# koszullab/instaGRAAL

Measured on AMD Instinct MI355X. Metric: MCMC moves/s (accepted+rejected) at fixed n_frags x nnz, higher is better.
Workload: dtype f32 screening tier with a rigorous bound (every column) + f64 terms (f32 inputs) for the contenders / exact i64 fixed-point sums; 1 GPU; synthetic Hi-C 50k bins / 50M contacts (149003 sub-frags), level 4, 5 neighbours, nuisance sampling off; seed=0, step=one batch of 128 moves (step_sampler calls), moves_warmup=640, parallelism=1 GPU, parameters=synthetic

## Files before the change

### include/instagraal_hip.h

```cpp
#ifndef INSTAGRAAL_HIP_H
#define INSTAGRAAL_HIP_H

#include <stdint.h>

#ifdef __cplusplus
extern "C" {
#endif

#define IG_N_TMP_STRUCT 24
#define IG_MAX_CANDIDATES 16
#define IG_N_INSERT_BLOCKS 6

typedef struct ig_ctx ig_ctx;

typedef struct ig_move_result {
    double o;
    double dist;
    double mean_len;
    int32_t op_sampled;
    int32_t id_f_sampled;
    int32_t n_contigs;
    int32_t n_candidates;
    int64_t n_slice;
    int64_t n_evals;
// ... 17 lines not shown
int ig_set_insert_config(ig_ctx* ctx, const int32_t list_bounds[IG_N_INSERT_BLOCKS], int32_t max_bounds_insert);
int ig_set_initial_genome(ig_ctx* ctx, const int32_t* init_prev, const int32_t* init_next, const int32_t* orientable,
                          const int32_t* blacklisted, int32_t n_blacklisted);

int ig_full_likelihood(ig_ctx* ctx, int which_params, int use_prev_tables, double* nz, double* z, int64_t* limbs5);

int ig_score_move(ig_ctx* ctx, int32_t frag_a, const int32_t* cands, int32_t C, double* scores);
int ig_apply(ig_ctx* ctx, int32_t frag_a, int32_t frag_b, int32_t op);
int ig_step(ig_ctx* ctx, int32_t frag_a, const int32_t* cands, int32_t C, ig_move_result* out, double* scores_or_null);
int ig_step_batch(ig_ctx* ctx, int32_t n_moves, const int32_t* frags, const int32_t* cands, int32_t max_c,
                  ig_move_result* results);
typedef struct ig_neighbours ig_neighbours;
int ig_neighbours_create(const int64_t* indptr, const int32_t* xk, const float* pk, int32_t n_frags, const int32_t* blacklisted,
                         int32_t n_blacklisted, ig_neighbours** out);
void ig_neighbours_destroy(ig_neighbours* nb);
int ig_neighbours_draw(ig_neighbours* nb, uint32_t* mt_key624, int32_t* mt_pos, const int32_t* frags, int32_t n_moves,
                       int32_t n_neighbours, int32_t* cands_out);
int ig_neighbours_draw_nuisance(ig_neighbours* nb, uint32_t* mt_key624, int32_t* mt_pos, int32_t* has_gauss, double* gauss,
                                const int32_t* frags, int32_t n_moves, int32_t n_neighbours, int32_t skip_normal_3, int32_t* cands_out,
                                int32_t* id_modif_out, double* normal_out, double* uniform_out);
int ig_step_draw(ig_ctx* ctx, ig_neighbours* nb, uint32_t* mt_key624, int32_t* mt_pos, int32_t frag_a, int32_t n_neighbours,
                 int32_t* cands, int32_t* n_cands, ig_move_result* out, double* scores_or_null);
int ig_step_batch_draw(ig_ctx* ctx, ig_neighbours* nb, uint32_t* mt_key624, int32_t* mt_pos, int32_t n_moves, const int32_t* frags,
                       int32_t n_neighbours, int32_t* cands_out, ig_move_result* results);
int ig_batch_max_width(ig_ctx* ctx, int32_t max_c);
int ig_batch_upload(ig_ctx* ctx, int32_t n_moves, const int32_t* frags, const int32_t* cands, int32_t max_c, int32_t max_w);
int ig_batch_score(ig_ctx* ctx, int32_t move0, int32_t W, int32_t slot_begin, int32_t slot_end);
int ig_batch_records(ig_ctx* ctx, void** records, int64_t* bytes_per_slot);
int ig_batch_commit(ig_ctx* ctx, int32_t move0, int32_t W, int32_t* n_committed);
int ig_batch_results(ig_ctx* ctx, int32_t n_moves, ig_move_result* results);
int ig_set_batch_width(int w);
int ig_set_window(int w);
int ig_batch_stats(ig_ctx* ctx, int64_t out4[4]);
int ig_scratch_bytes(ig_ctx* ctx, int64_t out3[3]);

int ig_nuis_begin(ig_ctx* ctx, int32_t frag_a, const int32_t* cands, int32_t C, const float p_test[8], float mean_subfrag_kb);
int ig_nuis_end(ig_ctx* ctx, ig_move_result* out, double* nz_test, double* z_test, int64_t* limbs5);
int ig_nuis_accept(ig_ctx* ctx);
int ig_links_inverse(ig_ctx* ctx);
int ig_set_nuis_width(int w);
int ig_nuis_run_begin(ig_ctx* ctx, int32_t n_moves, const int32_t* frags, const int32_t* cands, int32_t max_c);
int ig_nuis_step_begin(ig_ctx* ctx, int32_t move, const float p_test[8], float mean_subfrag_kb);
int ig_nuis_step_next(ig_ctx* ctx, double temperature, double u, const float p_next_rejected[8], const float p_next_accepted[8],
                      float mean_subfrag_kb, int32_t has_next, ig_move_result* out, double* nz_test, double* z_test, int32_t* accepted);
int ig_set_nuis_screen(int on);
int ig_set_nuis_hist(int on);
int ig_set_nuis_chain(int on);
int ig_nuis_chain_begin(ig_ctx* ctx, int32_t move, int32_t n_sets, const float* p_tests, const double* u, const double* temperature,
                        float mean_subfrag_kb);
int ig_nuis_chain_done(ig_ctx* ctx);
int ig_nuis_chain_end(ig_ctx* ctx, int32_t* n_done, int32_t* reason);
int ig_nuis_exact_result(ig_ctx* ctx, double* nz_test);

int ig_renumber_contigs(ig_ctx* ctx, int32_t* n_contigs, float* mean_len, int32_t* max_id);
int ig_bomb(ig_ctx* ctx, const int32_t* shuffle);
int ig_genome_distance(ig_ctx* ctx, double* d);
int ig_get_valid_insert(ig_ctx* ctx, int32_t out12[12]);

int ig_contact_map_order(ig_ctx* ctx, int32_t* order_M, int32_t* n_placed);
int ig_contact_map(ig_ctx* ctx, int32_t max_side, int64_t* image, int64_t image_capacity, int32_t* side, int32_t* bin);

int ig_distance_law(ig_ctx* ctx, const float* edges, int32_t n_edges, int64_t* observed, int64_t* pairs, int64_t scalars[8]);

int ig_set_shard(ig_ctx* ctx, int32_t rank, int32_t world);
int64_t ig_partials_count(ig_ctx* ctx);
void* ig_partials_device_ptr(ig_ctx* ctx);
// ... 39 lines not shown
```

### instagraal_amd/csrc/ig_common.cuh

```cuda
#pragma once

#include <hip/hip_runtime.h>

#include <algorithm>
#include <atomic>
#include <cstdarg>
#include <cstdio>
#include <cstdlib>
#include <cstring>
#include <numeric>
#include <string>
#include <vector>

#include "../../include/ig_detmath.h"
#include "../../include/instagraal_hip.h"
#include "ig_ops.cuh"

#define NSLOT 25
#define NCODE 8
#define NFRESH 4
#define LGF_TAB 1024
#define SCORE_THREADS 256

static thread_local std::string g_err;
// ... 11 lines not shown
#define HIPCK(x)                                                                                     \
    do {                                                                                             \
        hipError_t e_ = (x);                                                                         \
        if (e_ != hipSuccess) return fail("%s failed: %s (%s:%d)", #x, hipGetErrorString(e_), __FILE__, __LINE__); \
    } while (0)


struct SubTab {
    int parent;
    float wat, cri;
    int w;
};

struct State {
    int *pos, *spos, *cid, *sbp, *circ, *prev, *next, *L, *SL, *LB, *ori;
    int *lb, *sl, *sub_first, *rep, *activ, *id_d;
};
#define NDYN 11

struct Tables {
    float* dist;
    float* stot;
    int* len;
    int2* cp;
};

struct CandMeta {
    int B, ctgA, ctgB, same, windowed;
    int LA, LB, SLA, SLB, n_loc, m_loc;
    int lA, lB;
    int n_uniq, uniq[24], kidx[NSLOT];
    int flags[12], pos_up[6], pos_down[6];
    int pos_fa, pos_fb, up_fa, down_fa, up_fb, down_fb;
};

struct ColMeta {
    float stot;
    int len;
};

struct Glob {
    ig_params par[2];
    float mean_kb;
    int slice_nb;
    int list_bounds[6];
    long long nz_hi, nz_lo, z_hi, z_lo, n_intra;
    long long credit2, credit2_acc;
    double n_tot_pxl;
    double lgf[15];
    int n_contigs, next_cid, n_black, N, M;
    int max_L, max_SL;
    int n_prev_touched;
    int valid_insert[12];
    int error;
    int stamp_ctr;
    int retry_pool;
    int retry_pad;
    long long scr_cols, scr_cont;
    long long scr_void_cols;
    long long scr_terms, scr_terms_exact;
    int dbg[8];
};

#define IG_MAX_BATCH 64
struct MoveCtl {
    int A, C, force_slot, fresh;
    int ch_c, ch_k, ch_slot, ch_windowed;
    int superset0;
    int overflow;
    int n_dirty, pad;
    int exact_chunk, pad2;
    double ch_score;
    long long n_slice_tot, n_eval_tot, bytes_min;
    long long d_hi, d_lo;
    long long nzb_hi, nzb_lo;
    int pred, pred_c, pred_k, pred_pad;
    long long pd_hi, pd_lo;
};

struct SlotPre {
    long long nz_hi, nz_lo;
    double nz_d, nz_cut_d;
    long long dz_hi, dz_lo, dni;
    int k;
    unsigned info;
};
struct CandPre {
    long long ext_hi, ext_lo;
    double ext_d;
    long long n_slice;
    int r;
    int base_cnt;
    int ctgA, ctgB, m_loc, n_loc, n_uniq, B;
// ... 319 lines not shown
```

### instagraal_amd/csrc/ig_host_batch.inc

```


static int ensure_io(ig_ctx* c, int n_moves, int max_c)
{
    const size_t need = (size_t)n_moves * (sizeof(int) + (size_t)IG_MAX_CANDIDATES * sizeof(int) + sizeof(ig_move_result));
    if (c->h_stage_bytes < need) {
        if (c->h_stage) hipHostFree(c->h_stage);
        c->h_stage = nullptr;
        c->h_stage_bytes = 0;
        const size_t want = std::max(need, (size_t)1 << 20);
        if (hipHostMalloc((void**)&c->h_stage, want, hipHostMallocDefault) == hipSuccess) c->h_stage_bytes = want;
        else (void)hipGetLastError();
    }
    if (c->results_cap < n_moves) {
        const int cap = std::max(n_moves, 8192);
        hipFree(c->d_results);
        hipFree(c->d_frags);
        DALLOC(c->d_results, (size_t)cap);
        DALLOC(c->d_frags, (size_t)cap);
        c->results_cap = cap;
    }
    if ((long long)c->cands_cap < (long long)n_moves * max_c) {
        const long long cap = std::max((long long)n_moves * max_c, 8192LL * IG_MAX_CANDIDATES);
        hipFree(c->d_cands);
        DALLOC(c->d_cands, (size_t)cap);
// ... 111 lines not shown
    } stale_guard(c, par_only && pb > 0);
    const int N = c->N;
    const int gN = std::max((N + 255) / 256, W);
    const PzTab pz{c->pz_tab, c->pz_n};
    if (phase == 0 || phase == 2) {
        const int n_tw = (c->M + 31) / 32 + 1;
        if (!par_only) {
            c->touched_flip ^= 1;
            c->mb.touched = c->touched_bits + (size_t)c->touched_flip * n_tw;
        }
        if (!par_only) {
            const int mean_len0 = c->n_contigs_seen > 0 ? c->N / c->n_contigs_seen : 0;
            c->mb.nseg = mean_len0 >= 600 ? SLICE_SEG : 8;
        }
        if (!par_only) {
            TimedLaunch t(c, T_GATHER);
            hipLaunchKernelGGL(k_gather, dim3(gN), dim3(256), 0, c->stream, c->st, c->glob, c->mb, c->d_cands, c->d_frags, move0, W, max_c,
                               c->tab, c->tab_prev, c->prev_touched, force_slot, c->touched_bits + (size_t)(c->touched_flip ^ 1) * n_tw, n_tw);
        }
        if (!par_only) {
            TimedLaunch t(c, T_MUTATE);
            c->own_begin = w_begin;
            c->own_end = w_end;
            if (nW > 0) {
                const int mean_len = c->n_contigs_seen > 0 ? c->N / c->n_contigs_seen : 0;
                const int mutate_threads = mean_len >= 600 ? 1024 : (mean_len >= 150 ? 512 : 256);
                hipLaunchKernelGGL(k_mutate, dim3(NSLOT, max_c, nW), dim3(mutate_threads), 0, c->stream, c->st, c->tab, c->sub_tab, c->rowptr,
                                   c->glob, c->mb, pz, w_begin);
            }
        }
        if (force_slot < 0 && nW > 0) {
            if (!par_only) {
                TimedLaunch t(c, T_SLICE);
                hipLaunchKernelGGL(k_offsets, dim3(1), dim3(OFFSETS_THREADS), 0, c->stream, c->mb, W, w_begin, w_end, max_c);
                const int rb_auto = c->n_contigs_seen > 0
                                        ? std::min(SLICE_RB, std::max(32, (int)(2.0 * (double)c->Z / (double)c->n_contigs_seen / 2100.0)))
                                        : SLICE_RB;
                const int rb = nW == 1 ? std::max(rb_auto, 192) : rb_auto;
                const int s_share = 1, s_maxj = 1 << 20;
                if (c->mb.packed)
                    hipLaunchKernelGGL(k_slice<true>, dim3(rb, max_c + 1, nW), dim3(256), 0, c->stream, c->rowptr, c->cc, c->tab, c->glob, c->mb, c->rank,
                                       c->world, w_begin, s_share, s_maxj);
                else
                    hipLaunchKernelGGL(k_slice<false>, dim3(rb, max_c + 1, nW), dim3(256), 0, c->stream, c->rowptr, c->cc, c->tab, c->glob, c->mb, c->rank,
                                       c->world, w_begin, s_share, s_maxj);
            }
            if (par_only && nWp > 0)
                hipLaunchKernelGGL(k_rescore_prepare, dim3(NSLOT, max_c, nWp), dim3(256), 0, c->stream, c->glob, c->mb, pz, pb);
            if (nWp > 0) {
            const int s_screen = getenv("IG_SCREEN") ? atoi(getenv("IG_SCREEN")) : 1;
            const int verify = getenv("IG_SCREEN_VERIFY") ? atoi(getenv("IG_SCREEN_VERIFY")) : 0;
            const bool exact_once = c->exact_next && !par_only;
            if (exact_once) c->exact_next = false;
            const bool screen = (s_screen || verify) && phase == 2 && (W > 1 || c->screen_w1) && c->world == 1 && c->mb.packed && !exact_once;
            c->tail_fused = screen;
            if (phase == 2 && !c->tail_fused) {
                hipEventRecord(c->ev_slice, c->stream);
                hipStreamWaitEvent(c->stream2, c->ev_slice, 0);
                hipLaunchKernelGGL(k_tail, dim3(max_c, nWp), dim3(256), 0, c->stream2, c->rowptr, c->cc, c->tab, c->glob, c->mb, c->lgf_tab,
                                   g_tail_quirk, pz, pb);
                hipEventRecord(c->ev_tail, c->stream2);
            }
            int contenders_only = 0;
            if (screen) {
                const int ny = (NSLOT + 1) / 2;
                const int use_order = (!par_only && pb == w_begin && pe == w_end && nWp * max_c <= (int)OFFSETS_THREADS) ? 1 : 0;
                const int nseg = c->mb.nseg;
                const int Q = std::max(1, std::min(8, (7000 + nseg * ny * max_c * nWp - 1) / (nseg * ny * max_c * nWp)));
                {
                    TimedLaunch t(c, T_SCREEN);
                    const int tsplit = (nWp == 1 && !par_only) ? 6 : 1;
                    if (c->tail_fused)
                        hipLaunchKernelGGL(k_screen_tail, dim3(max_c * nWp * tsplit + nseg * Q * ny * max_c * nWp), dim3(SCORE_THREADS), 0, c->stream,
                                           c->screen_const, c->mb, c->mb.scr, c->mb.scr_void, c->mb.scr_ub, max_c, pb, max_c * nWp * tsplit, c->rowptr, c->cc,
                                           c->tab, c->glob, c->lgf_tab, g_tail_quirk, pz, use_order, Q, tsplit);
                    else
                        hipLaunchKernelGGL(k_screen<0>, dim3(nseg * Q, ny, max_c * nWp), dim3(SCORE_THREADS), 0, c->stream, c->screen_const,
                                           c->mb, c->mb.scr, c->mb.scr_void, c->mb.scr_ub, max_c, pb, use_order, Q);
// ... 639 lines not shown
    if (n_moves < 0 || n_moves > c->up_moves) return fail("ig_batch_results: out of range");
    return download_results(c, n_moves, results);
}

extern "C" int ig_set_batch_width(int w)
{
    g_batch_w = std::min(std::max(w, 1), IG_MAX_BATCH);
    return 0;
}

extern "C" int ig_scratch_bytes(ig_ctx* c, int64_t out3[3])
{
    IG_JOIN(c);
    const MoveBuf& m = c->mb;
    const int64_t C = (int64_t)m.capC * m.capW;
    out3[0] = C * ((int64_t)m.sN * 4 * 3 + (int64_t)m.sM * 4 * 2 + (int64_t)m.sM * NSLOT * 8 + (int64_t)NSLOT * NDYN * m.sN * 4);
    out3[1] = m.pool_cap * (m.packed ? 8 : 12);
    out3[2] = C * (int64_t)(SLICE_SEG * 16 + sizeof(CandMeta) + NSLOT * NCODE * sizeof(ColMeta) + (P_STRIDE + Q_STRIDE) * 8 + IG_N_TMP_STRUCT * 8 +
                            NSLOT * 8 + NSLOT * 16 + 16) +
              (int64_t)m.rec_stride * m.capW + (int64_t)m.work_cap * 8 + (int64_t)c->N * 8;
    return 0;
}

extern "C" int ig_batch_stats(ig_ctx* c, int64_t out3[4])
{
    IG_JOIN(c);
    out3[0] = c->n_batches;
    out3[1] = c->n_batch_committed;
    out3[2] = c->n_batch_pending;
    out3[3] = c->n_batch_predicted;
    return 0;
}

extern "C" int ig_step(ig_ctx* c, int32_t frag_a, const int32_t* cands, int32_t C, ig_move_result* out, double* scores)
{
    IG_JOIN(c);
    HIPCK(hipSetDevice(c->device));
    if (check_ready(c)) return -1;
    if (c->world > 1) return fail("ig_step: this handle scores a contact shard (ig_set_shard %d/%d): partial sums only -- use ig_step_begin / all-reduce / ig_step_finish", c->rank, c->world);
    if (validate_move(c, frag_a, cands, C)) return -1;
    if (ensure_move_buffers(c, std::max(8, (int)C))) return -1;
    if (ensure_io(c, 1, C)) return -1;
    char* stg = (c->h_stage && c->h_stage_bytes >= 8192) ? (char*)c->h_stage : nullptr;
    int* s_in = stg ? (int*)stg : nullptr;
    ig_move_result* s_res = stg ? (ig_move_result*)(stg + 256) : out;
    double* s_sc = stg ? (double*)(stg + 512) : scores;
    if (s_in) {
        s_in[0] = frag_a;
        for (int i = 0; i < C; i++) s_in[1 + i] = cands[i];
    }
    HIPCK(hipMemcpyAsync(c->d_frags, s_in ? (const void*)s_in : (const void*)&frag_a, sizeof(int), hipMemcpyHostToDevice, c->stream));
    HIPCK(hipMemcpyAsync(c->d_cands, s_in ? (const void*)(s_in + 1) : (const void*)cands, (size_t)C * sizeof(int), hipMemcpyHostToDevice, c->stream));
    for (;;) {
        enqueue_move(c, 0, C, -1, 2);
        if (scores) HIPCK(hipMemcpyAsync(s_sc, c->mb.scores, (size_t)C * IG_N_TMP_STRUCT * sizeof(double), hipMemcpyDeviceToHost, c->stream));
        enqueue_apply(c, 0, 0, 0);
        HIPCK(hipMemcpyAsync(s_res, c->d_results, sizeof(ig_move_result), hipMemcpyDeviceToHost, c->stream));
        if (queue_max_readback(c)) return -1;
        HIPCK(hipStreamSynchronize(c->stream));
        if (s_res->pad != 1) break;
        take_max_readback(c);
        if (retry_with_larger_pool(c)) return -1;
    }
    if (stg) {
        *out = *s_res;
        if (scores) memcpy(scores, s_sc, (size_t)C * IG_N_TMP_STRUCT * sizeof(double));
// ... 280 lines not shown
```

### instagraal_amd/csrc/ig_kernels_score.cuh

```cuda
#pragma once


#define CW(w, c) (PS(w) * mb.capC + (c))

__device__ inline int build_uniq(int* u, bool first, int LA, int LB, const int* vf)
{
    int n = 0;
    if (first) {
        u[n++] = 0;
        u[n++] = 1;
    }
    u[n++] = 2;
    u[n++] = 3;
    if (LB != 1)
        for (int k = 4; k < 8; k++) u[n++] = k;
    if (LA != 1)
        for (int k = 8; k < 12; k++) u[n++] = k;
    for (int k = 12; k < IG_N_TMP_STRUCT; k++)
        if (!vf || vf[k - 12] != -1) u[n++] = k;
    return n;
}

__global__ void __launch_bounds__(256)
    k_gather(State st, Glob* g, MoveBuf mb, const int* __restrict__ cands_all, const int* __restrict__ frags_all, int move0, int W,
// ... 281 lines not shown
        for (int x = threadIdx.x; x < n; x += blockDim.x) {
            const int f = S.gid[x];
            ch |= (S.pos[x] != st.pos[f]) | (S.spos[x] != st.spos[f]) | (S.cid[x] != st.cid[f]) | (S.sbp[x] != st.sbp[f]) |
                  (S.circ[x] != st.circ[f]) | (S.prev[x] != st.prev[f]) | (S.next[x] != st.next[f]) | (S.L[x] != st.L[f]) |
                  (S.SL[x] != st.SL[f]) | (S.LB[x] != st.LB[f]) | (S.ori[x] != st.ori[f]);
            hd += (S.pos[x] == 0);
            if (in_lds) {
#pragma unroll
                for (int a = 0; a < NDYN; a++) base[(size_t)a * N + x] = s_loc[a * MUT_LDS_N + x];
            }
        }
        __shared__ int sh_ch, sh_hd;
        if (threadIdx.x == 0) {
            sh_ch = 0;
            sh_hd = 0;
        }
        __syncthreads();
        hd = wave_sum_i(hd);
        if ((threadIdx.x & 63) == 0 && hd) atomicAdd(&sh_hd, hd);
        if (ch) atomicOr(&sh_ch, 1);
        __syncthreads();
        if (threadIdx.x == 0) {
            mb.sinfo[cw * NSLOT + slot] = make_int2(sh_ch, sh_hd);
            if (sh_ch && k > 0) atomicOr(&mb.livecol[cw], 1u << k);
        }
    }
    const ig_params p = g->par[0];
    const float mean = g->mean_kb;
    uint2* col = mb.coords + (size_t)(cw * NSLOT + k) * M;
    ColMeta* cm = mb.cmeta + (size_t)(cw * NSLOT + k) * NCODE;
    int* subs = mb.subs + (size_t)cw * M;
    long long hi = 0, lo = 0, ni = 0;
    __shared__ long long seg_bound[SLICE_SEG];
    if (threadIdx.x < SLICE_SEG) seg_bound[threadIdx.x] = 0;
    __syncthreads();
    for (int x = threadIdx.x; x < n; x += blockDim.x) {
        const int f = S.gid[x];
        const int cid = S.cid[x];
        const int code = (cid == m.ctgA) ? 0 : ((cid == m.ctgB) ? 1 : 2 + (cid - fresh));
        const int ori = S.ori[x], sp = S.spos[x], sl = S.sl[x], SLc = S.SL[x];
        const float stot = (float)(int)((float)S.circ[x] * (float)S.LB[x] / 1000.0f);
        if (S.pos[x] == 0) {
            cm[code].stot = stot;
            cm[code].len = SLc;
        }
        const float sbp_kb = (float)S.sbp[x] / 1000.0f;
        const int sf = st.sub_first[f];
        const int lbase = (x < m.LA) ? 0 : m.SLA;
        for (int q = 0; q < sl; q++) {
            const int s = sf + q;
            const SubTab b = sub[s];
            const float dist = sbp_kb + ((ori == 1) ? b.wat : b.cri);
            const int npos = (ori == 1) ? sp + q : sp + sl - (q + 1);
            const int ls = lbase + tab.cp[s].y;
            uint2 v;
            v.x = __float_as_uint(dist);
            v.y = (unsigned)npos | ((unsigned)code << 28);
            col[ls] = v;
            if (k == 0) {
                subs[ls] = s;
                mb.rowcnt[(size_t)cw * M + ls] = 0;
                const long long rb = rowptr[s], re = rowptr[s + 1];
                atomicAdd((unsigned long long*)&seg_bound[ls & (mb.nseg - 1)], (unsigned long long)(re - rb));
                mb.rowbe[(size_t)cw * M + ls] = make_int4((int)(unsigned)rb, (int)(rb >> 32), (int)(re - rb), s);
            }
            if (npos == 0) ni += ((long long)SLc * (long long)(SLc - 1)) / 2;
            if (npos > 0) {
                const long long q2 = zero_q(p, npos, SLc, stot, mean, pz.v, pz.n);
                hi += q2 >> 32;
                lo += (long long)(unsigned int)q2;
            }
        }
    }
    __shared__ long long red[4][16];
    hi = wave_sum_ll(hi);
    lo = wave_sum_ll(lo);
    ni = wave_sum_ll(ni);
    const int wv = threadIdx.x >> 6;
    if ((threadIdx.x & 63) == 0) {
        red[0][wv] = hi;
        red[1][wv] = lo;
        red[2][wv] = ni;
    }
    __syncthreads();
    if (threadIdx.x == 0) {
        long long* q = mb.qpart + (size_t)cw * Q_STRIDE;
        long long s0 = 0, s1 = 0, s2 = 0;
        for (int v = 0; v < (int)(blockDim.x >> 6); v++) {
            s0 += red[0][v];
            s1 += red[1][v];
            s2 += red[2][v];
        }
        q[Q_Z + 2 * k] = s0;
        q[Q_Z + 2 * k + 1] = s1;
        q[Q_NI + k] = s2;
    }
    if (k == 0 && threadIdx.x < SLICE_SEG) mb.slbound[(size_t)cw * SLICE_SEG + threadIdx.x] = seg_bound[threadIdx.x];
}

__global__ void __launch_bounds__(1024) k_mutate(State st, Tables tab, const SubTab* __restrict__ sub, const long long* __restrict__ rowptr,
                                                Glob* g, MoveBuf mb, PzTab pz, int w_begin)
{
    if (KEPT(w_begin + (int)blockIdx.z)) return;
    mutate_one(st, tab, sub, rowptr, g, mb, pz, blockIdx.x, blockIdx.y, w_begin + blockIdx.z);
}

__global__ void __launch_bounds__(256) k_mutate_winners(State st, Tables tab, const SubTab* __restrict__ sub,
                                                        const long long* __restrict__ rowptr, Glob* g, MoveBuf mb, PzTab pz, int w_start,
                                                        int own_begin, int own_end, const int* __restrict__ batch_out)
{
    const int w = blockIdx.y;
    const int committed = batch_out[0], pending = batch_out[1];
    if (w >= own_begin && w < own_end) return;
    if (!((w >= w_start && w < committed) || w == pending)) return;
    const MoveCtl& mc = mb.ctl[PS(w)];
    if (blockIdx.x == 1 && mc.ch_slot == IG_N_TMP_STRUCT) return;
    mutate_one(st, tab, sub, rowptr, g, mb, pz, blockIdx.x == 0 ? IG_N_TMP_STRUCT : mc.ch_slot, mc.ch_c, w);
}

#define OFFSETS_THREADS 1024
__global__ void __launch_bounds__(OFFSETS_THREADS) k_offsets(MoveBuf mb, int W, int w_begin, int w_end, int max_c)
{
    __shared__ long long wave_tot[OFFSETS_THREADS / 64];
    __shared__ long long s_tot[IG_MAX_BATCH * IG_MAX_CANDIDATES];
    const int tid = threadIdx.x, lane = tid & 63, wv = tid >> 6;
    const int n_idx = (w_end - w_begin) * max_c;
    const bool can_order = n_idx <= IG_MAX_BATCH * IG_MAX_CANDIDATES && n_idx <= (int)OFFSETS_THREADS;
    long long my_tot = 0;
    if (can_order && tid < n_idx) {
        const int w = w_begin + tid / max_c, c = tid % max_c;
        const bool used = c < mb.ctl[PS(w)].C && !KEPT(w);
        for (int sg = 0; sg < SLICE_SEG; sg++) {
            const long long b = mb.slbound[(size_t)CW(w, c) * SLICE_SEG + sg];
            my_tot += (used && b > 0) ? b : 0;
        }
    }
    const int n = W * mb.capC * SLICE_SEG;
    const int per = (n + OFFSETS_THREADS - 1) / OFFSETS_THREADS;
    auto phys = [&](int i) -> size_t {
        const int cwl = i / SLICE_SEG;
        return (size_t)CW(cwl / mb.capC, cwl % mb.capC) * SLICE_SEG + (size_t)(i % SLICE_SEG);
    };
    auto bound_of = [&](int i) -> long long {
        const int cwl = i / SLICE_SEG;
        const int w = cwl / mb.capC, c = cwl % mb.capC;
        return (w >= w_begin && w < w_end && !KEPT(w) && c < mb.ctl[PS(w)].C) ? mb.slbound[phys(i)] : -1;
    };
    constexpr int PER_MAX = (IG_MAX_BATCH * IG_MAX_CANDIDATES * SLICE_SEG + OFFSETS_THREADS - 1) / OFFSETS_THREADS;
    long long bq[PER_MAX];
    __shared__ int s_over[IG_MAX_BATCH];
    if (tid < IG_MAX_BATCH) s_over[tid] = 0;
    long long sum = 0;
#pragma unroll
    for (int q = 0; q < PER_MAX; q++) {
        const int i = tid * per + q;
        bq[q] = (q < per && i < n) ? bound_of(i) : -1;
        sum += bq[q] > 0 ? bq[q] : 0;
    }
    long long incl = sum;
    for (int off = 1; off < 64; off <<= 1) {
        const long long o = __shfl_up(incl, off, 64);
        if (lane >= off) incl += o;
    }
    if (lane == 63) wave_tot[wv] = incl;
    __syncthreads();
    long long run = incl - sum;
    for (int q = 0; q < wv; q++) run += wave_tot[q];
#pragma unroll
    for (int q = 0; q < PER_MAX; q++) {
        const int i = tid * per + q;
        const long long b = bq[q];
        if (b >= 0) {
            if (run + b > mb.pool_cap) {
                mb.sloff[phys(i)] = -1;
                mb.ctl[PS(i / SLICE_SEG / mb.capC)].overflow = 1;
                s_over[i / SLICE_SEG / mb.capC] = 1;
            } else {
                mb.sloff[phys(i)] = run;
            }
            run += b;
        }
    }
    __syncthreads();
#pragma unroll
    for (int q = 0; q < PER_MAX; q++) {
        const int i = tid * per + q;
        if (bq[q] >= 0 && s_over[i / SLICE_SEG / mb.capC]) mb.sloff[phys(i)] = -1;
    }
    if (can_order) {
        if (tid < n_idx) s_tot[tid] = my_tot;
        __syncthreads();
        if (tid < n_idx) {
            int rank = 0;
            for (int u = 0; u < n_idx; u++) rank += (s_tot[u] > my_tot) || (s_tot[u] == my_tot && u < tid);
            mb.order[rank] = ((w_begin + tid / max_c) << 8) | (tid % max_c);
        }
        const int n_slots = w_end - w_begin;
        long long st = 0;
        if (tid < n_slots)
            for (int cc2 = 0; cc2 < max_c; cc2++) st += s_tot[tid * max_c + cc2];
        __syncthreads();
        if (tid < n_slots) s_tot[tid] = st;
        __syncthreads();
        if (tid < n_slots) {
            int rank = 0;
            for (int u = 0; u < n_slots; u++) rank += (s_tot[u] > st) || (s_tot[u] == st && u < tid);
            mb.order[mb.capC * mb.capW + rank] = w_begin + tid;
        }
    } else if (tid < w_end - w_begin) {
        mb.order[mb.capC * mb.capW + tid] = w_begin + tid;
    }
}

#define LDS_COL_CAP 4096
#define DELTA_RB 128

#ifndef SLICE_RB
#define SLICE_RB 96
#endif
#ifndef SLICE_UNROLL
#define SLICE_UNROLL 4
#endif
#ifndef SLICE_MIN_WAVES
#define SLICE_MIN_WAVES 8
#endif
template <bool PACKED>
__global__ void __launch_bounds__(256, SLICE_MIN_WAVES) k_slice(const long long* __restrict__ rowptr, const int2* __restrict__ cc, Tables tab,
                                                                 Glob* g, MoveBuf mb, int rank, int world, int w_begin, int share_rows, int max_j)
{
    const int w = mb.order[mb.capC * mb.capW + blockIdx.z];
    if (KEPT(w)) return;
    const bool shared_plane = (blockIdx.y == 0);
    const int cand_plane = (int)blockIdx.y - 1;
    __shared__ long long seg_off[IG_MAX_CANDIDATES][SLICE_SEG];
    __shared__ int s_cw[IG_MAX_CANDIDATES], s_ctgB[IG_MAX_CANDIDATES], s_idx[IG_MAX_CANDIDATES], s_nc;
    __shared__ int a_same[IG_MAX_CANDIDATES], a_ctgB[IG_MAX_CANDIDATES], a_SLA, a_ctgA, a_mloc[IG_MAX_CANDIDATES];
    const int lane = threadIdx.x & 63, wv = threadIdx.x >> 6;
    const unsigned long long lt_mask = (1ull << lane) - 1ull;
    const int C = mb.ctl[PS(w)].C;
    const int capC = min(mb.capC, IG_MAX_CANDIDATES);
    if ((int)threadIdx.x < capC) {
        const CandMeta& mt = mb.meta[CW(w, threadIdx.x)];
        a_same[threadIdx.x] = mt.same;
        a_ctgB[threadIdx.x] = mt.ctgB;
        a_mloc[threadIdx.x] = mt.m_loc;
        if (threadIdx.x == 0) {
            a_SLA = mt.SLA;
            a_ctgA = mt.ctgA;
        }
    }
    for (int i = threadIdx.x; i < capC * SLICE_SEG; i += blockDim.x) seg_off[i / SLICE_SEG][i % SLICE_SEG] = mb.sloff[(size_t)CW(w, i / SLICE_SEG) * SLICE_SEG + i % SLICE_SEG];
    __syncthreads();
    if (threadIdx.x == 0) {
        int nc = 0;
        if (shared_plane) {
            if (share_rows)
                for (int c = 0; c < C; c++)
                    if (!a_same[c]) {
                        s_idx[nc] = c;
                        s_cw[nc] = CW(w, c);
                        s_ctgB[nc++] = a_ctgB[c];
                    }
        } else if (cand_plane < C) {
            s_idx[0] = cand_plane;
            s_cw[0] = CW(w, cand_plane);
            s_ctgB[0] = a_ctgB[cand_plane];
            nc = 1;
        }
        s_nc = nc;
    }
    __syncthreads();
    const int nc = s_nc;
    if (nc == 0) return;
    if (seg_off[0][0] < 0) return;
    const int cw0 = s_cw[0], c0 = s_idx[0];
    const CandMeta& m = mb.meta[cw0];
    const int M = mb.sM;
    const bool m_same = a_same[c0] != 0;
    const bool own_all = !shared_plane && (m_same || !share_rows);
    const int SLA = a_SLA, ctgA = a_ctgA;
    const int row_lo = (shared_plane || own_all) ? 0 : SLA;
    const int n_rows = shared_plane ? SLA : (a_mloc[c0] - row_lo);
    const int4* rowbe = mb.rowbe + (size_t)cw0 * M;
    const int ctgB0 = s_ctgB[0];
    const int nrw = gridDim.x * 4;
    const int J = min(max_j, max(1, nrw / max(n_rows, 1)));
    for (int item = blockIdx.x * 4 + wv; item < n_rows * J; item += nrw) {
        const int r = row_lo + item % n_rows, j = item / n_rows;
        const int seg = r & (mb.nseg - 1);
        const int4 be = rowbe[r];
        const long long b = (long long)(unsigned)be.x | ((long long)be.y << 32), e = b + be.z;
        const bool in_a = m_same || r < SLA;
        const int2 cp1 = make_int2(in_a ? ctgA : ctgB0, in_a ? r : r - SLA);
        const bool mine = (world <= 1) || ((r % world) == rank);
        int rc = 0;
        if (b != e) {
            for (long long q0 = b + (long long)j * 64 * SLICE_UNROLL; q0 < e; q0 += (long long)J * 64 * SLICE_UNROLL) {
                int2 v[SLICE_UNROLL], cp2[SLICE_UNROLL];
#pragma unroll
                for (int u = 0; u < SLICE_UNROLL; u++) {
                    const long long qi = q0 + u * 64 + lane;
                    v[u] = (qi < e) ? cc[qi] : make_int2(-1, 0);
                }
#pragma unroll
                for (int u = 0; u < SLICE_UNROLL; u++) {
                    const bool hit = (v[u].x >= 0) && ((mb.touched[v[u].x >> 5] >> (v[u].x & 31)) & 1u);
                    cp2[u] = hit ? tab.cp[v[u].x] : make_int2(-1, -1);
                }
                for (int k = 0; k < nc; k++) {
                    bool keep[SLICE_UNROLL];
                    unsigned long long mask[SLICE_UNROLL];
                    int add = 0;
                    const int ctgB = s_ctgB[k];
#pragma unroll
                    for (int u = 0; u < SLICE_UNROLL; u++) {
                        if (own_all) keep[u] = (v[u].x >= 0) && slice_keep(m, cp1.x, cp2[u].x, cp1.y, cp2[u].y, v[u].y, false);
                        else keep[u] = (v[u].x >= 0) && (v[u].y > 0) && ((cp2[u].x == ctgA) || (cp2[u].x == ctgB));
                        mask[u] = __ballot(keep[u]);
                        add += __popcll(mask[u]);
                    }
                    if (!add) continue;
                    rc += (lane == k) ? add : 0;
                    if (!mine) continue;
                    unsigned long long base = 0;
                    if (lane == 0) base = atomicAdd((unsigned long long*)(mb.part + (size_t)s_cw[k] * P_STRIDE + P_CNT + seg), (unsigned long long)add);
                    base = __shfl(base, 0, 64);
                    const long long off = seg_off[s_idx[k]][seg];
                    int o2 = 0;
#pragma unroll
                    for (int u = 0; u < SLICE_UNROLL; u++) {
                        if (keep[u]) {
                            const long long at = off + (long long)base + o2 + __popcll(mask[u] & lt_mask);
                            const int lj = ((m_same || cp2[u].x == ctgA) ? 0 : SLA) + cp2[u].y;
                            if (PACKED) {
                                mb.sl_pk[at] = (unsigned long long)r | ((unsigned long long)lj << 20) | ((unsigned long long)v[u].y << 40);
                            } else {
                                mb.sl_li[at] = r;
                                mb.sl_lj[at] = lj;
                                mb.sl_ob[at] = v[u].y;
                            }
                        }
                        o2 += __popcll(mask[u]);
                    }
                }
            }
        }
        if (lane < nc && rc) atomicAdd(&mb.rowcnt[(size_t)s_cw[lane] * M + r], rc);
    }
}

#define LDS_PZ 1024
#define LDS_LGF 256

__device__ __noinline__ double term_general(const ig_params p, float mean_kb, float s, int dkey, int ob, double lgf, PzTab pz)
{
    const ig_hot h = ig_hot_make(p, ig_tab());
    const int inter = dkey < 0;
    const float ex_z = inter ? p.v_inter : pz_lookup(pz, p, mean_kb, dkey);
    if (h.fast && ob > 0) return ig_term_hot(s, inter, ob, lgf, ex_z, &h, ig_tab());
    const float ex = inter ? p.v_inter : ig_rippe(s, p, ig_tab());
    return ig_pixel_term(ex, ex_z, ob, lgf, ig_tab());
}

__device__ __forceinline__ void quantize_split(double t, int& qh, unsigned& ql)
{
    t = (t != t) ? 0.0 : t;
// ... 1322 lines not shown
```

### instagraal_amd/hip_lib.py

```python
from __future__ import annotations

import ctypes as C
import os
import subprocess

import numpy as np

HERE = os.path.dirname(os.path.abspath(__file__))
ROOT = os.path.dirname(HERE)
LIB_PATH = os.path.join(HERE, "libinstagraal_hip.so")
SRC = os.path.join(HERE, "csrc", "ig_hip.hip")
SRC_HOST = os.path.join(HERE, "csrc", "ig_draw.cpp")
DEPS = [SRC, SRC_HOST] + [os.path.join(HERE, "csrc", f) for f in ("ig_ops.cuh", "ig_common.cuh", "ig_model.cuh", "ig_kernels_setup.cuh",
                                                          "ig_kernels_score.cuh", "ig_kernels_screen.cuh", "ig_kernels_commit.cuh",
                                                          "ig_kernels_nuis.cuh", "ig_kernels_map.cuh", "ig_kernels_law.cuh", "ig_host_core.inc", "ig_host_upload.inc",
                                                          "ig_host_map.inc", "ig_host_law.inc",
                                                          "ig_host_batch.inc", "ig_host_nuis.inc", "ig_host_debug.inc")] + \
       [os.path.join(ROOT, "include", f) for f in ("ig_detmath.h", "ig_detmath_tables.h", "instagraal_hip.h")]

N_TMP_STRUCT = 24
MAX_CANDIDATES = 16

FRAG_FIELDS = ("pos", "sub_pos", "id_c", "start_bp", "len_bp", "sub_len", "circ", "id", "prev", "next", "l_cont",
               "sub_l_cont", "l_cont_bp", "ori", "rep", "activ", "id_d")
# ... 483 lines not shown
        o = np.zeros(12, np.float64)
        _ck(lib().ig_debug_nuis_screen_stats(self._h, _p(o)))
        n = max(o[0] - o[3], 1.0)
        return dict(screened=int(o[0]), rejected_screened=int(o[1]), exact_passes=int(o[2]), void=int(o[3]), largest_bound=float(o[4]),
                    largest_used_fraction=float(o[5]), mean_bound=float(o[6] / n), undecided=int(o[7]),
                    void_why=dict(parameters=int(o[8]), contact=int(o[9]), sums=int(o[10]), no_record=int(o[11])))

    def debug_nuis_hist_stats(self):
        o = np.zeros(12, np.float64)
        _ck(lib().ig_debug_nuis_hist_stats(self._h, _p(o)))
        n = max(o[0] - o[3], 1.0)
        return dict(evaluated=int(o[0]), rejected=int(o[1]), accepted=int(o[2]), void=int(o[3]), mean_bound=float(o[4] / n),
                    largest_used_fraction=float(o[5]), walks=int(o[6]), builds=int(o[7]),
                    void_why=dict(parameters=int(o[8]), contact=int(o[9]), sums=int(o[10]), no_record=int(o[11])))

    def debug_zero_fallbacks(self):
        n = C.c_int64()
        _ck(lib().ig_debug_zero_fallbacks(self._h, C.byref(n)))
        return int(n.value)

    def debug_pool_retries(self):
        n = C.c_int64()
        _ck(lib().ig_debug_pool_retries(self._h, C.byref(n)))
        return int(n.value)

    def debug_nuis_hist_check(self):
        n = C.c_int64()
        _ck(lib().ig_debug_nuis_hist_check(self._h, C.byref(n)))
        return int(n.value)

    def batch_stats(self):
        o = np.zeros(4, np.int64)
        _ck(lib().ig_batch_stats(self._h, _p(o)))
        return dict(batches=int(o[0]), committed_in_batch=int(o[1]), one_move_tails=int(o[2]), predicted_deltas=int(o[3]))

    def scratch_bytes(self):
        o = np.zeros(3, np.int64)
        _ck(lib().ig_scratch_bytes(self._h, _p(o)))
        return int(o[0]), int(o[1]), int(o[2])

    def contact_map_order(self):
        out = np.zeros(max(self.M, 1), np.int32)
        n = C.c_int32()
        _ck(lib().ig_contact_map_order(self._h, _p(out), C.byref(n)))
        return out[:n.value].copy()

    def contact_map(self, max_side):
        from .contact_map import binning

        max_side = int(max_side)
        if not 1 <= max_side <= 2 ** 31 - 1:
            raise HipError("contact_map: max_side must be >= 1 (got %d)" % max_side)
        cap = min(max_side, max(self.M, 1))
        if cap * cap > 1 << 26:
            cap = max(binning(self.contact_map_order().size, max_side)[1], 1)
        img = np.empty(cap * cap, np.int64)
        side, b = C.c_int32(), C.c_int32()
        _ck(lib().ig_contact_map(self._h, C.c_int32(max_side), _p(img), C.c_int64(img.size), C.byref(side), C.byref(b)))
        n = side.value
        return img[:n * n].reshape(n, n).copy(), b.value

    def debug_contact_map_time(self, max_side, combine=True, n=1):
        ms = np.zeros(int(n), np.float32)
        tot = C.c_int64()
        _ck(lib().ig_debug_contact_map_time(self._h, C.c_int32(int(max_side)), C.c_int32(int(bool(combine))), C.c_int32(int(n)), _p(ms),
                                            C.byref(tot)))
        return ms, int(tot.value)
# ... 139 lines not shown
```

Measured before the change: 51960 moves/s.

## Share slice row walks among candidates with same target contig, add walk stats

```diff
diff --git a/include/instagraal_hip.h b/include/instagraal_hip.h
--- a/include/instagraal_hip.h
+++ b/include/instagraal_hip.h
@@ -73,6 +73,7 @@
 int ig_set_batch_width(int w);
 int ig_set_window(int w);
 int ig_batch_stats(ig_ctx* ctx, int64_t out4[4]);
+int ig_slice_walk_stats(ig_ctx* ctx, int64_t out2[2]);
 int ig_scratch_bytes(ig_ctx* ctx, int64_t out3[3]);
 
 int ig_nuis_begin(ig_ctx* ctx, int32_t frag_a, const int32_t* cands, int32_t C, const float p_test[8], float mean_subfrag_kb);
diff --git a/instagraal_amd/csrc/ig_common.cuh b/instagraal_amd/csrc/ig_common.cuh
--- a/instagraal_amd/csrc/ig_common.cuh
+++ b/instagraal_amd/csrc/ig_common.cuh
@@ -67,6 +67,7 @@
     int n_uniq, uniq[24], kidx[NSLOT];
     int flags[12], pos_up[6], pos_down[6];
     int pos_fa, pos_fb, up_fa, down_fa, up_fb, down_fb;
+    int rows_a;
 };
 
 struct ColMeta {
@@ -94,6 +95,7 @@
     long long scr_cols, scr_cont;
     long long scr_void_cols;
     long long scr_terms, scr_terms_exact;
+    long long slice_walked, slice_walked_per_cand;
     int dbg[8];
 };
 
diff --git a/instagraal_amd/csrc/ig_host_batch.inc b/instagraal_amd/csrc/ig_host_batch.inc
--- a/instagraal_amd/csrc/ig_host_batch.inc
+++ b/instagraal_amd/csrc/ig_host_batch.inc
@@ -167,18 +167,18 @@
         if (force_slot < 0 && nW > 0) {
             if (!par_only) {
                 TimedLaunch t(c, T_SLICE);
-                hipLaunchKernelGGL(k_offsets, dim3(1), dim3(OFFSETS_THREADS), 0, c->stream, c->mb, W, w_begin, w_end, max_c);
+                hipLaunchKernelGGL(k_offsets, dim3(1), dim3(OFFSETS_THREADS), 0, c->stream, c->mb, c->glob, W, w_begin, w_end, max_c);
                 const int rb_auto = c->n_contigs_seen > 0
-                                        ? std::min(SLICE_RB, std::max(32, (int)(2.0 * (double)c->Z / (double)c->n_contigs_seen / 2100.0)))
+                                        ? std::min(SLICE_RB, std::max(32, (int)(2.0 * (double)c->Z / (double)c->n_contigs_seen / SLICE_RB_CONTACTS)))
                                         : SLICE_RB;
                 const int rb = nW == 1 ? std::max(rb_auto, 192) : rb_auto;
-                const int s_share = 1, s_maxj = 1 << 20;
+                const int s_maxj = 1 << 20;
                 if (c->mb.packed)
                     hipLaunchKernelGGL(k_slice<true>, dim3(rb, max_c + 1, nW), dim3(256), 0, c->stream, c->rowptr, c->cc, c->tab, c->glob, c->mb, c->rank,
-                                       c->world, w_begin, s_share, s_maxj);
+                                       c->world, w_begin, s_maxj);
                 else
                     hipLaunchKernelGGL(k_slice<false>, dim3(rb, max_c + 1, nW), dim3(256), 0, c->stream, c->rowptr, c->cc, c->tab, c->glob, c->mb, c->rank,
-                                       c->world, w_begin, s_share, s_maxj);
+                                       c->world, w_begin, s_maxj);
             }
             if (par_only && nWp > 0)
                 hipLaunchKernelGGL(k_rescore_prepare, dim3(NSLOT, max_c, nWp), dim3(256), 0, c->stream, c->glob, c->mb, pz, pb);
@@ -884,6 +884,18 @@
     return 0;
 }
 
+extern "C" int ig_slice_walk_stats(ig_ctx* c, int64_t out2[2])
+{
+    IG_JOIN(c);
+    HIPCK(hipSetDevice(c->device));
+    HIPCK(hipStreamSynchronize(c->stream));
+    long long h[2] = {0, 0};
+    HIPCK(hipMemcpy(h, (const char*)c->glob + offsetof(Glob, slice_walked), sizeof h, hipMemcpyDeviceToHost));
+    out2[0] = h[0];
+    out2[1] = h[1];
+    return 0;
+}
+
 extern "C" int ig_step(ig_ctx* c, int32_t frag_a, const int32_t* cands, int32_t C, ig_move_result* out, double* scores)
 {
     IG_JOIN(c);
diff --git a/instagraal_amd/csrc/ig_kernels_score.cuh b/instagraal_amd/csrc/ig_kernels_score.cuh
--- a/instagraal_amd/csrc/ig_kernels_score.cuh
+++ b/instagraal_amd/csrc/ig_kernels_score.cuh
@@ -337,7 +337,9 @@
     int* subs = mb.subs + (size_t)cw * M;
     long long hi = 0, lo = 0, ni = 0;
     __shared__ long long seg_bound[SLICE_SEG];
+    __shared__ int rows_a;
     if (threadIdx.x < SLICE_SEG) seg_bound[threadIdx.x] = 0;
+    if (threadIdx.x == 0) rows_a = 0;
     __syncthreads();
     for (int x = threadIdx.x; x < n; x += blockDim.x) {
         const int f = S.gid[x];
@@ -367,6 +369,7 @@
                 mb.rowcnt[(size_t)cw * M + ls] = 0;
                 const long long rb = rowptr[s], re = rowptr[s + 1];
                 atomicAdd((unsigned long long*)&seg_bound[ls & (mb.nseg - 1)], (unsigned long long)(re - rb));
+                if (ls < m.SLA) atomicAdd(&rows_a, (int)(re - rb));
                 mb.rowbe[(size_t)cw * M + ls] = make_int4((int)(unsigned)rb, (int)(rb >> 32), (int)(re - rb), s);
             }
             if (npos == 0) ni += ((long long)SLc * (long long)(SLc - 1)) / 2;
@@ -401,6 +404,7 @@
         q[Q_NI + k] = s2;
     }
     if (k == 0 && threadIdx.x < SLICE_SEG) mb.slbound[(size_t)cw * SLICE_SEG + threadIdx.x] = seg_bound[threadIdx.x];
+    if (k == 0 && threadIdx.x == 0) mb.meta[cw].rows_a = rows_a;
 }
 
 __global__ void __launch_bounds__(1024) k_mutate(State st, Tables tab, const SubTab* __restrict__ sub, const long long* __restrict__ rowptr,
@@ -424,7 +428,7 @@
 }
 
 #define OFFSETS_THREADS 1024
-__global__ void __launch_bounds__(OFFSETS_THREADS) k_offsets(MoveBuf mb, int W, int w_begin, int w_end, int max_c)
+__global__ void __launch_bounds__(OFFSETS_THREADS) k_offsets(MoveBuf mb, Glob* g, int W, int w_begin, int w_end, int max_c)
 {
     __shared__ long long wave_tot[OFFSETS_THREADS / 64];
     __shared__ long long s_tot[IG_MAX_BATCH * IG_MAX_CANDIDATES];
@@ -432,9 +436,16 @@
     const int n_idx = (w_end - w_begin) * max_c;
     const bool can_order = n_idx <= IG_MAX_BATCH * IG_MAX_CANDIDATES && n_idx <= (int)OFFSETS_THREADS;
     long long my_tot = 0;
+    int my_ctgA = -1, my_ctgB = -1, my_rows_a = 0;
     if (can_order && tid < n_idx) {
         const int w = w_begin + tid / max_c, c = tid % max_c;
         const bool used = c < mb.ctl[PS(w)].C && !KEPT(w);
+        if (c < mb.capC) {
+            const CandMeta& mt = mb.meta[CW(w, c)];
+            my_ctgA = mt.ctgA;
+            my_ctgB = used ? mt.ctgB : -1;
+            my_rows_a = mt.rows_a;
+        }
         for (int sg = 0; sg < SLICE_SEG; sg++) {
             const long long b = mb.slbound[(size_t)CW(w, c) * SLICE_SEG + sg];
             my_tot += (used && b > 0) ? b : 0;
@@ -493,8 +504,33 @@
         if (bq[q] >= 0 && s_over[i / SLICE_SEG / mb.capC]) mb.sloff[phys(i)] = -1;
     }
     if (can_order) {
-        if (tid < n_idx) s_tot[tid] = my_tot;
+        __shared__ int s_cB[IG_MAX_BATCH * IG_MAX_CANDIDATES];
+        if (tid < n_idx) {
+            s_tot[tid] = my_tot;
+            s_cB[tid] = my_ctgB;
+        }
         __syncthreads();
+        if (tid < n_idx && tid % max_c == 0 && my_ctgB >= 0 && !s_over[(w_begin + tid / max_c)]) {
+            long long walked = my_rows_a, per_cand = 0;
+            bool other = false;
+            for (int c = 0; c < max_c; c++) {
+                const int cB = s_cB[tid + c];
+                if (cB < 0) continue;
+                if (cB == my_ctgA) {
+                    per_cand += my_rows_a;
+                    continue;
+                }
+                other = true;
+                const long long rows_b = s_tot[tid + c] - my_rows_a;
+                per_cand += rows_b;
+                bool first = true;
+                for (int c2 = 0; c2 < c; c2++) first = first && (s_cB[tid + c2] != cB);
+                if (first) walked += rows_b;
+            }
+            if (other) per_cand += my_rows_a;
+            atomic_add_ll(&g->slice_walked, walked);
+            atomic_add_ll(&g->slice_walked_per_cand, per_cand);
+        }
         if (tid < n_idx) {
             int rank = 0;
             for (int u = 0; u < n_idx; u++) rank += (s_tot[u] > my_tot) || (s_tot[u] == my_tot && u < tid);
@@ -523,6 +559,9 @@
 #ifndef SLICE_RB
 #define SLICE_RB 96
 #endif
+#ifndef SLICE_RB_CONTACTS
+#define SLICE_RB_CONTACTS 2100.0
+#endif
 #ifndef SLICE_UNROLL
 #define SLICE_UNROLL 4
 #endif
@@ -531,72 +570,75 @@
 #endif
 template <bool PACKED>
 __global__ void __launch_bounds__(256, SLICE_MIN_WAVES) k_slice(const long long* __restrict__ rowptr, const int2* __restrict__ cc, Tables tab,
-                                                                 Glob* g, MoveBuf mb, int rank, int world, int w_begin, int share_rows, int max_j)
+                                                                 Glob* g, MoveBuf mb, int rank, int world, int w_begin, int max_j)
 {
     const int w = mb.order[mb.capC * mb.capW + blockIdx.z];
     if (KEPT(w)) return;
-    const bool shared_plane = (blockIdx.y == 0);
     const int cand_plane = (int)blockIdx.y - 1;
     __shared__ long long seg_off[IG_MAX_CANDIDATES][SLICE_SEG];
-    __shared__ int s_cw[IG_MAX_CANDIDATES], s_ctgB[IG_MAX_CANDIDATES], s_idx[IG_MAX_CANDIDATES], s_nc;
-    __shared__ int a_same[IG_MAX_CANDIDATES], a_ctgB[IG_MAX_CANDIDATES], a_SLA, a_ctgA, a_mloc[IG_MAX_CANDIDATES];
+    __shared__ int s_cw[IG_MAX_CANDIDATES], s_ctgB[IG_MAX_CANDIDATES], s_idx[IG_MAX_CANDIDATES], s_won[IG_MAX_CANDIDATES];
+    __shared__ int4 s_win[IG_MAX_CANDIDATES];
+    __shared__ int s_nc, s_focal, s_share, s_part, s_rows, a_SLA, a_ctgA;
     const int lane = threadIdx.x & 63, wv = threadIdx.x >> 6;
     const unsigned long long lt_mask = (1ull << lane) - 1ull;
     const int C = mb.ctl[PS(w)].C;
     const int capC = min(mb.capC, IG_MAX_CANDIDATES);
-    if ((int)threadIdx.x < capC) {
-        const CandMeta& mt = mb.meta[CW(w, threadIdx.x)];
-        a_same[threadIdx.x] = mt.same;
-        a_ctgB[threadIdx.x] = mt.ctgB;
-        a_mloc[threadIdx.x] = mt.m_loc;
-        if (threadIdx.x == 0) {
-            a_SLA = mt.SLA;
-            a_ctgA = mt.ctgA;
+    if (wv == 0) {
+        const bool have = lane < capC && lane < C;
+        int same = 0, ctgB = -1, mloc = 0, won = 0, SLA = 0, ctgA = -1;
+        int4 win = make_int4(0, 0, 0, 0);
+        if (have) {
+            const CandMeta& mt = mb.meta[CW(w, lane)];
+            same = mt.same;
+            ctgB = mt.ctgB;
+            mloc = mt.m_loc;
+            won = mt.windowed;
+            win = make_int4(mt.up_fa, mt.down_fa, mt.up_fb, mt.down_fb);
+            SLA = mt.SLA;
+            ctgA = mt.ctgA;
+        }
+        const int cp = min(max(cand_plane, 0), 63);
+        const int p_same = __shfl(same, cp, 64), p_ctgB = __shfl(ctgB, cp, 64);
+        const bool focal = cand_plane < 0 || cand_plane >= C || p_same != 0;
+        const bool served = have && (focal || ctgB == p_ctgB);
+        const bool walker = lane < (int)gridDim.y - 1 && (focal ? (lane >= C || same != 0) : (have && ctgB == p_ctgB));
+        const unsigned long long m_served = __ballot(served), m_walker = __ballot(walker);
+        if (served) {
+            const int at = __popcll(m_served & lt_mask);
+            s_idx[at] = lane;
+            s_cw[at] = CW(w, lane);
+            s_ctgB[at] = ctgB;
+            s_won[at] = won;
+            s_win[at] = win;
+            if (at == 0) s_rows = focal ? SLA : mloc - SLA;
+        }
+        if (lane == 0) {
+            s_nc = __popcll(m_served);
+            s_focal = focal ? 1 : 0;
+            s_share = __popcll(m_walker) + (focal ? 1 : 0);
+            s_part = cand_plane < 0 ? 0 : __popcll(m_walker & ((1ull << cp) - 1ull)) + (focal ? 1 : 0);
+            a_SLA = SLA;
+            a_ctgA = ctgA;
         }
     }
     for (int i = threadIdx.x; i < capC * SLICE_SEG; i += blockDim.x) seg_off[i / SLICE_SEG][i % SLICE_SEG] = mb.sloff[(size_t)CW(w, i / SLICE_SEG) * SLICE_SEG + i % SLICE_SEG];
-    __syncthreads();
-    if (threadIdx.x == 0) {
-        int nc = 0;
-        if (shared_plane) {
-            if (share_rows)
-                for (int c = 0; c < C; c++)
-                    if (!a_same[c]) {
-                        s_idx[nc] = c;
-                        s_cw[nc] = CW(w, c);
-                        s_ctgB[nc++] = a_ctgB[c];
-                    }
-        } else if (cand_plane < C) {
-            s_idx[0] = cand_plane;
-            s_cw[0] = CW(w, cand_plane);
-            s_ctgB[0] = a_ctgB[cand_plane];
-            nc = 1;
-        }
-        s_nc = nc;
-    }
     __syncthreads();
     const int nc = s_nc;
     if (nc == 0) return;
     if (seg_off[0][0] < 0) return;
-    const int cw0 = s_cw[0], c0 = s_idx[0];
-    const CandMeta& m = mb.meta[cw0];
     const int M = mb.sM;
-    const bool m_same = a_same[c0] != 0;
-    const bool own_all = !shared_plane && (m_same || !share_rows);
+    const bool focal = s_focal != 0;
     const int SLA = a_SLA, ctgA = a_ctgA;
-    const int row_lo = (shared_plane || own_all) ? 0 : SLA;
-    const int n_rows = shared_plane ? SLA : (a_mloc[c0] - row_lo);
-    const int4* rowbe = mb.rowbe + (size_t)cw0 * M;
-    const int ctgB0 = s_ctgB[0];
-    const int nrw = gridDim.x * 4;
+    const int row_lo = focal ? 0 : SLA;
+    const int n_rows = s_rows;
+    const int4* rowbe = mb.rowbe + (size_t)s_cw[0] * M;
+    const int nrw = gridDim.x * 4 * s_share;
     const int J = min(max_j, max(1, nrw / max(n_rows, 1)));
-    for (int item = blockIdx.x * 4 + wv; item < n_rows * J; item += nrw) {
+    for (int item = (s_part * gridDim.x + blockIdx.x) * 4 + wv; item < n_rows * J; item += nrw) {
         const int r = row_lo + item % n_rows, j = item / n_rows;
         const int seg = r & (mb.nseg - 1);
         const int4 be = rowbe[r];
         const long long b = (long long)(unsigned)be.x | ((long long)be.y << 32), e = b + be.z;
-        const bool in_a = m_same || r < SLA;
-        const int2 cp1 = make_int2(in_a ? ctgA : ctgB0, in_a ? r : r - SLA);
         const bool mine = (world <= 1) || ((r % world) == rank);
         int rc = 0;
         if (b != e) {
@@ -617,10 +659,15 @@
                     unsigned long long mask[SLICE_UNROLL];
                     int add = 0;
                     const int ctgB = s_ctgB[k];
+                    const bool won = s_won[k] != 0;
+                    const int4 wn = s_win[k];
 #pragma unroll
                     for (int u = 0; u < SLICE_UNROLL; u++) {
-                        if (own_all) keep[u] = (v[u].x >= 0) && slice_keep(m, cp1.x, cp2[u].x, cp1.y, cp2[u].y, v[u].y, false);
-                        else keep[u] = (v[u].x >= 0) && (v[u].y > 0) && ((cp2[u].x == ctgA) || (cp2[u].x == ctgB));
+                        keep[u] = (v[u].x >= 0) && (v[u].y > 0) && ((cp2[u].x == ctgA) || (cp2[u].x == ctgB));
+                        if (won) {
+                            const int px = min(r, cp2[u].y), py = max(r, cp2[u].y);
+                            keep[u] = keep[u] && (((px <= wn.y) && (py >= wn.x)) || ((py >= wn.z) && (px <= wn.w)));
+                        }
                         mask[u] = __ballot(keep[u]);
                         add += __popcll(mask[u]);
                     }
@@ -636,7 +683,7 @@
                     for (int u = 0; u < SLICE_UNROLL; u++) {
                         if (keep[u]) {
                             const long long at = off + (long long)base + o2 + __popcll(mask[u] & lt_mask);
-                            const int lj = ((m_same || cp2[u].x == ctgA) ? 0 : SLA) + cp2[u].y;
+                            const int lj = ((cp2[u].x == ctgA) ? 0 : SLA) + cp2[u].y;
                             if (PACKED) {
                                 mb.sl_pk[at] = (unsigned long long)r | ((unsigned long long)lj << 20) | ((unsigned long long)v[u].y << 40);
                             } else {
diff --git a/instagraal_amd/hip_lib.py b/instagraal_amd/hip_lib.py
--- a/instagraal_amd/hip_lib.py
+++ b/instagraal_amd/hip_lib.py
@@ -539,7 +539,10 @@
     def batch_stats(self):
         o = np.zeros(4, np.int64)
         _ck(lib().ig_batch_stats(self._h, _p(o)))
-        return dict(batches=int(o[0]), committed_in_batch=int(o[1]), one_move_tails=int(o[2]), predicted_deltas=int(o[3]))
+        w = np.zeros(2, np.int64)
+        _ck(lib().ig_slice_walk_stats(self._h, _p(w)))
+        return dict(batches=int(o[0]), committed_in_batch=int(o[1]), one_move_tails=int(o[2]), predicted_deltas=int(o[3]),
+                    slice_contacts_walked=int(w[0]), slice_contacts_walked_per_candidate=int(w[1]))
 
     def scratch_bytes(self):
         o = np.zeros(3, np.int64)
```

After: 53510 moves/s (median of 6 runs). +3.0%, better.
